# okieraised/rs-face-detection-tflite

Measured on AMD Instinct MI355X. Metric: faces/sec at batch=256 (256x256 back-camera) per GPU, higher is better.
Workload: dtype f32

## Files before the change

rs-face-detection-tflite_amd/csrc/engine.cpp:

```cpp
#include "engine.hpp"
#include "launch.hpp"

#include <algorithm>
#include <cstdio>
#include <cstdlib>
#include <cstring>
#include <stdexcept>

namespace mi {

void hip_check(hipError_t e, const char* what) {
    if (e != hipSuccess) throw std::runtime_error(std::string(what) + ": " + hipGetErrorString(e));
}

namespace {
template <class T>
void upload(T*& dev, std::vector<T>& host, const char* what_alloc, const char* what_copy) {
    if (dev) hip_check(hipFree(dev), "hipFree");
    dev = nullptr;
    if (host.empty()) return;
    hip_check(hipMalloc(reinterpret_cast<void**>(&dev), host.size() * sizeof(T)), what_alloc);
    hip_check(hipMemcpy(dev, host.data(), host.size() * sizeof(T), hipMemcpyHostToDevice), what_copy);
    std::vector<T>().swap(host);
}
}

Model::Model(const uint8_t* bytes, size_t n, int device) : device_(device), blob_(bytes, bytes + n) {
    int count = 0;
    if (hipGetDeviceCount(&count) != hipSuccess || count <= 0)
        throw std::runtime_error("no HIP device visible: the MI355X kernels cannot run (no CPU fallback exists)");
    if (device < 0 || device >= count) throw std::runtime_error("device ordinal out of range");
    hip_check(hipSetDevice(device_), "hipSetDevice");
    hipDeviceProp_t prop;
    hip_check(hipGetDeviceProperties(&prop, device_), "hipGetDeviceProperties");
    if (std::string(prop.gcnArchName).rfind("gfx950", 0) != 0)
        throw std::runtime_error(std::string("kernels are built for gfx950 only; device is ") + prop.gcnArchName);
    hip_check(hipStreamCreateWithFlags(&stream_, hipStreamNonBlocking), "hipStreamCreate");
    rebuild();
}

Model::~Model() {
    hipSetDevice(device_);
    invalidate_graphs();
    if (d_weights_) hipFree(d_weights_);
    if (d_programs_) hipFree(d_programs_);
    if (d_tail_programs_) hipFree(d_tail_programs_);
    if (d_arena_) hipFree(d_arena_);
    if (d_small_) hipFree(d_small_);
    if (d_in_stage_) hipFree(d_in_stage_);
    free_bandnet();
    for (float* p : d_out_)
        if (p) hipFree(p);
    for (hipStream_t st : side_streams_) hipStreamDestroy(st);
    for (hipEvent_t ev : lane_events_) hipEventDestroy(ev);
    for (hipStream_t st : head_streams_) hipStreamDestroy(st);
    for (hipEvent_t ev : head_events_) if (ev) hipEventDestroy(ev);
    if (stream_) hipStreamDestroy(stream_);
}

void Model::invalidate_graphs() {
    if (!graphs_.empty()) (void)hipDeviceSynchronize();
    for (auto& kv : graphs_) hipGraphExecDestroy(kv.second);
    graphs_.clear();
}

struct Model::Option {
    enum { kReplan = 1,
           kFreeSmall = 2,
           kKeepGraphs = 4,
           kOneOf = 8,
           kKiB = 16 , kWriteOnly = 32, kReadOnly = 64,
           kBandGen = 128 };
    const char* key;
    int Model::*field;
    int lo, hi, flags;
};

const Model::Option* Model::find_option(const std::string& key) {
    using O = Option;
    constexpr int kMax = 0x7fffffff;
    static const Option table[] = {
        {"chunk", &Model::chunk_, 0, kMax, 0},
        {"graph", &Model::use_graph_, 0, 1, 0},
        {"fuse", &Model::fuse_level_, 0, 5, O::kReplan},
        {"res_budget", &Model::res_budget_, 16, 156, O::kReplan | O::kKiB},
        {"pipe", &Model::pipe_max_, 0, 4, O::kReplan},
        {"small_chain", &Model::small_chain_, 0, 64, O::kFreeSmall},
        {"pipe_rows", &Model::pipe_rows_, 1 << 1 | 1 << 2 | 1 << 4, 0, O::kOneOf},
        {"pipe_band", &Model::pipe_band_, 0, 4096, 0},
        {"strip", &Model::strip_, 0, 1, 0},
        {"stem_fuse", &Model::stem_fuse_, 0, 1, 0},
        {"stem_mfma", &Model::stem_mfma_, 0, 1, 0},
        {"pair_fuse", &Model::pair_fuse_, 0, 1, 0},
        {"mdb_band", &Model::mdb_band_, 0, 4096, 0},
        {"mchain", &Model::mchain_, 0, 1, 0},
        {"tail", &Model::tail_, 0, 1, O::kReplan},
        {"tail_pre", &Model::tail_pre_, 0, 2, 0},
        {"tail_g", &Model::tail_g_, 0, 64, 0},
        {"band", &Model::band_, 0, 2, O::kReplan},
        {"band_test_fail", &Model::band_test_fail_, 0, 1, O::kWriteOnly},
        {"band_test_absent", &Model::band_test_absent_, 0, 256, O::kWriteOnly},
        {"band_test_gen", nullptr, 0, kMax, O::kBandGen | O::kWriteOnly},
        {"band_wide", &Model::band_wide_ok_, 0, 1, O::kReplan},
        {"band_fork", &Model::band_fork_, 0, 1, O::kReplan},
        {"band_nw", &Model::band_nw_, 8, 256, O::kReplan},
        {"band_fail_streak", &Model::band_fail_streak_, 0, 0, O::kReadOnly},
        {"band_wraps", &Model::band_wraps_, 0, 0, O::kReadOnly},
        {"fork", &Model::fork_, 0, 1, 0},
        {"heads", &Model::head_streams_opt_, 1, kHeadStreams, O::kReplan},
        {"reuse", &Model::reuse_, 0, 1, O::kReplan},
        {"lanes", &Model::lanes_, 1, 4, 0},
        {"test_poison", &Model::test_poison_, 1 << 1 | 1 << 2, 0, O::kOneOf | O::kKeepGraphs},
    };
    for (const Option& o : table)
        if (key == o.key) return &o;
    return nullptr;
}

void Model::set_option(const std::string& key, int value) {
    const Option* o = find_option(key);
    if (!o || (o->flags & Option::kReadOnly)) throw std::runtime_error("unknown option '" + key + "'");
    int v = (o->lo == 0 && o->hi == 1) ? value != 0 : std::min(o->hi, std::max(o->lo, value));
    if (o->flags & Option::kOneOf) v = (value >= 0 && value < 31 && (o->lo >> value & 1)) ? value : 0;
    if (o->flags & Option::kKiB) v *= 1024;
    if (o->flags & Option::kBandGen) { band_gen_ = static_cast<unsigned>(v); band_gen_force_ = true; }
    else this->*o->field = v;
    if (o->flags & Option::kKeepGraphs) return;
    if (o->flags & Option::kReplan) dirty_ = true;
    if ((o->flags & Option::kFreeSmall) && d_small_) { hipFree(d_small_); d_small_ = nullptr; small_floats_ = 0; }
    invalidate_graphs();
    chunk_cap_ = 0;
}

int Model::get_option(const std::string& key) const {
    const Option* o = find_option(key);
    if (!o || (o->flags & Option::kWriteOnly)) throw std::runtime_error("unknown option '" + key + "'");
    const int v = this->*o->field;
    return (o->flags & Option::kKiB) ? v / 1024 : v;
}

void Model::rebuild() {
    if (d_small_) { hipFree(d_small_); d_small_ = nullptr; small_floats_ = 0; }
    hip_check(hipSetDevice(device_), "hipSetDevice");
    invalidate_graphs();
    plan_ = build_plan(parse_tflite(blob_.data(), blob_.size()), fuse_level_, pipe_max_, res_budget_, tail_ != 0);
    if (!reuse_) {
        long off = 0;
        for (size_t t = 0; t < plan_.graph.tensors.size(); t++)
            if (plan_.root_offset[t] >= 0) { plan_.root_offset[t] = off; off += plan_.root_elems[t]; }
        plan_.arena_floats_per_frame = off;
    }
    consts_ = pack_plan_consts(plan_);
    upload(d_weights_, consts_.blob, "hipMalloc weights", "upload weights");
    upload(d_tail_programs_, consts_.tail_progs, "hipMalloc programs", "upload programs");
    upload(d_programs_, consts_.progs, "hipMalloc programs", "upload programs");
    sched_ = schedule_side_streams(plan_, head_streams_opt_);
    build_bandnet();
    dirty_ = false;
    chunk_cap_ = 0;
}

void Model::free_bandnet() {
    if (d_band_prog_) hipFree(d_band_prog_);
    if (d_band_consts_) hipFree(d_band_consts_);
    if (d_band_ws_) hipFree(d_band_ws_);
    if (d_band_sync_) hipFree(d_band_sync_);
    if (h_band_fail_) hipHostFree(h_band_fail_);
    d_band_prog_ = nullptr; d_band_consts_ = nullptr; d_band_ws_ = nullptr; d_band_sync_ = nullptr; h_band_fail_ = nullptr; d_band_fail_ = nullptr;
    band_plan_ = BandPlan();
}

void Model::build_bandnet() {
    free_bandnet();
    if (!band_ || fuse_level_ < 2) return;
    BandOptions o;
    o.nw = band_nw_; o.wide = band_wide_ok_ != 0; o.fork = band_fork_ != 0; o.cu_count = device_cu_count();
// ... 97 lines not shown
        for (int c : {n.w, n.b, n.w2, n.b2, n.alpha}) weights += 4 * elems(c);
        double bytes = per_frame * batch + weights;
        const auto& si = g.tensors[n.in[0]].shape;
        const auto& so = g.tensors[n.out].shape;
        if (n.kind == Node::Conv) macs = elems(n.out) * n.KH * n.KW * si.back() * batch;
        if (n.kind == Node::Dw) macs = elems(n.out) * n.KH * n.KW * batch;
        if (n.kind == Node::Block) macs = elems(n.out) / so.back() * si.back() * ((n.w >= 0 ? 9 : 0) + so.back()) * batch;
        if (n.kind == Node::Resident) {
            for (int t : n.extra_out) bytes += 4 * elems(t) * batch;
            for (const Node& m : n.members) {
                const auto& mo = g.tensors[m.out].shape;
                const int Cm = g.tensors[m.in[0]].shape[3];
                if (m.kind == Node::Conv) macs += elems(m.out) * m.KH * m.KW * Cm * batch;
                else macs += static_cast<double>(mo[1]) * mo[2] * Cm * ((m.w >= 0 ? 9 : 0) + mo[3]) * batch;
                for (int c : {m.w, m.b, m.w2, m.b2, m.alpha}) bytes += 4 * elems(c);
            }
        }
        if (n.kind == Node::Chain) {
            for (int t : n.extra_out) bytes += 4 * elems(t) * batch;
            for (const Node& m : n.members) {
                const auto& mo = g.tensors[m.out].shape;
                macs += static_cast<double>(mo[1]) * mo[2] * g.tensors[m.in[0]].shape[3] * (9 + mo[3]) * batch;
            }
            for (const Node& m : n.members)
                for (int c : {m.w, m.b, m.w2, m.b2, m.alpha}) bytes += 4 * elems(c);
            for (const Node& m : n.head_nodes) {
                macs += elems(m.out) * g.tensors[m.in[0]].shape[3] * batch;
                for (int c : {m.w, m.b, m.w2, m.b2}) bytes += 4 * elems(c);
            }
        }
        st.bytes += bytes;
        st.macs += macs;
        auto dims = [](const std::vector<int>& sh) {
            std::string d;
            for (size_t q = 1; q < sh.size(); q++) d += (q > 1 ? "x" : "") + std::to_string(sh[q]);
            return d;
        };
        if (static_cast<int>(i) == first.launches[k].node) st.detail = dims(si) + "->";
        st.detail = st.detail.substr(0, st.detail.find("->") + 2) + dims(so);
    }
    return stats;
}

LaunchCtx Model::launch_ctx(const float* in, int chunk_start, int frames) const {
    LaunchCtx c;
    c.weights = d_weights_;
    c.arena = d_arena_ + static_cast<size_t>(plan_.arena_floats_per_frame) * chunk_cap_ * arena_lane_;
    c.in = in; c.out = d_out_.data();
    c.small = d_small_; c.small_floats = small_floats_;
    c.progs = d_programs_; c.tail_progs = d_tail_programs_;
    c.band_prog = d_band_prog_; c.band_consts = d_band_consts_; c.band_ws = d_band_ws_; c.band_sync = d_band_sync_; c.band_fail = d_band_fail_;
    c.chunk_cap = chunk_cap_; c.chunk_start = chunk_start; c.F = frames;
    c.u8_frames = u8_.frames; c.u8_lut = u8_.lut; c.u8_frame_bytes = u8_.frame_bytes; c.u8_row_bytes = u8_.row_bytes;
    c.strip = strip_; c.pair_fuse = pair_fuse_; c.stem_fuse = stem_fuse_; c.stem_mfma = stem_mfma_; c.mchain = mchain_;
    c.small_chain = small_chain_; c.lanes = lanes_;
    c.pipe_rows = pipe_rows_; c.pipe_band = pipe_band_; c.mdb_band = mdb_band_; c.tail_pre = tail_pre_; c.tail_g = tail_g_;
    c.fork = fork_ && lanes_ == 1;
    c.cu_count = device_cu_count();
    c.band = band_use_ && chunk_start == 0;
    c.band_test_absent = band_test_absent_;
    return c;
}

namespace {
int issue(const Launch& l, hipStream_t s) {
    auto many = [&](int (*f)(const BlockArgs*, int, void*)) { return f(l.blocks.data(), static_cast<int>(l.blocks.size()), s); };
    switch (l.to) {
        case Launcher::Conv: return launch_conv(std::get<ConvArgs>(l.args), s);
        case Launcher::HeadGemm: return launch_head_gemm(std::get<HeadGemmArgs>(l.args), s);
        case Launcher::Dw: return launch_dw(std::get<DwArgs>(l.args), s);
        case Launcher::Xc: return launch_xc(std::get<XcArgs>(l.args), s);
        case Launcher::Mdblock: return launch_mdblock(std::get<DblockArgs>(l.args), s);
        case Launcher::Dblock: return launch_dblock(std::get<DblockArgs>(l.args), s);
        case Launcher::Mbneck: return launch_mbneck(std::get<BneckArgs>(l.args), s);
        case Launcher::Bneck: return launch_bneck(std::get<BneckArgs>(l.args), s);
        case Launcher::Tail: return launch_tail(std::get<TailLaunch>(l.args), s);
        case Launcher::Resident: return launch_resident(std::get<ResLaunch>(l.args), s);
        case Launcher::Chain: return launch_chain(std::get<ChainArgs>(l.args), s);
        case Launcher::StripPipe: return many(launch_strip_pipe);
        case Launcher::MstripChain: return many(launch_mstrip_chain);
        case Launcher::SmallChain: {
            int rc = 0;
            for (size_t k = 0; k < l.blocks.size() && rc == 0; k++) rc = l.blocks[k].sh == 1 ? launch_strip(l.blocks[k], s) : launch_block(l.blocks[k], s);
            return rc;
        }
        case Launcher::Ms2: return launch_ms2(std::get<BlockArgs>(l.args), s);
        case Launcher::Mwalk: return launch_mwalk(std::get<BlockArgs>(l.args), s);
        case Launcher::Strip: return launch_strip(std::get<BlockArgs>(l.args), s);
        case Launcher::Mstrip: return launch_mstrip(std::get<BlockArgs>(l.args), s);
        case Launcher::Block: return launch_block(std::get<BlockArgs>(l.args), s);
        case Launcher::Add: return launch_add(std::get<EltArgs>(l.args), s);
        case Launcher::Act: return launch_act(std::get<EltArgs>(l.args), s);
        case Launcher::Maxpool: return launch_maxpool(std::get<EltArgs>(l.args), s);
        case Launcher::Padc: return launch_padc(std::get<EltArgs>(l.args), s);
        case Launcher::Resize2x: return launch_resize2x(std::get<EltArgs>(l.args), s);
        case Launcher::DepthToSpace: return launch_depth_to_space(std::get<EltArgs>(l.args), s);
        case Launcher::Bandnet: return launch_bandnet(std::get<BandLaunch>(l.args), s);
    }
    return 0;
}
}

void Model::enqueue_chunk(const float* in, int chunk_start, int F, hipStream_t trunk, std::vector<hipEvent_t>* marks, Lowered* keep) {
    LaunchCtx ctx = launch_ctx(in, chunk_start, F);
    if (marks) ctx.fork = false;
    Lowered low = lower_chunk(plan_, consts_, band_plan_, sched_, ctx, keep != nullptr);
    auto mark = [&] {
// ... 254 lines not shown
```

rs-face-detection-tflite_amd/csrc/engine.hpp:

```cpp
#pragma once

#include <hip/hip_runtime.h>

#include <map>
#include <memory>
#include <string>
#include <vector>

#include "bandplan.hpp"
#include "consts.hpp"
#include "launches.hpp"
#include "plan.hpp"

namespace mi {

void hip_check(hipError_t e, const char* what);

class Model {
   public:
    Model(const uint8_t* bytes, size_t n, int device);
    ~Model();
    Model(const Model&) = delete;
    Model& operator=(const Model&) = delete;

    int device() const { return device_; }
    const Graph& graph() const { return plan_.graph; }
    const Plan& plan() const { return plan_; }
    std::vector<int> input_dims() const { return plan_.graph.tensors[plan_.graph.inputs[0]].shape; }
    int num_outputs() const { return static_cast<int>(plan_.graph.outputs.size()); }
    const std::vector<int>& output_dims(int i) const { return plan_.graph.tensors[plan_.graph.outputs.at(i)].shape; }
    size_t output_elems(int i) const { return plan_.graph.tensors[plan_.graph.outputs.at(i)].elems(); }
    size_t input_elems() const { return plan_.graph.tensors[plan_.graph.inputs[0]].elems(); }

    void run_device(const float* in, int batch, hipStream_t stream, bool one_shot = false);
    bool band_failed();
    int get_option(const std::string& key) const;
    int band_workgroups(int batch);
    void run(const float* in, int batch, float* const* outs, int mem, hipStream_t stream);
    float* output_device(int i) const { return d_out_.at(i); }
    hipStream_t stream() const { return stream_; }
    bool takes_u8_input();
    void run_device_u8(const uint8_t* frames, long frame_bytes, int row_bytes, const float* lut, int batch, hipStream_t stream);

    struct LaunchStat {
        std::string kernel, detail;
        double ms = 0, bytes = 0, macs = 0;
    };
    std::vector<LaunchStat> profile(const float* in, int batch, int reps, hipStream_t stream);
    void set_option(const std::string& key, int value);
    size_t debug_tensor(int tensor, int frame, float* dst, size_t cap);
    std::string describe() const { return plan_.describe(); }

   private:
    void rebuild();
    struct Option;
    static const Option* find_option(const std::string& key);
    void build_bandnet();
    void free_bandnet();
    bool band_usable(int batch) const;
    void band_before_launch(hipStream_t s);
    void poison_scratch(hipStream_t s);
    void ensure_capacity(int batch);
    LaunchCtx launch_ctx(const float* in, int chunk_start, int frames) const;
    void enqueue_chunk(const float* in, int chunk_start, int frames, hipStream_t s, std::vector<hipEvent_t>* marks = nullptr, Lowered* keep = nullptr);
    void enqueue_all(const float* in, int batch, hipStream_t s);
    void invalidate_graphs();

    int device_ = 0;
    std::vector<uint8_t> blob_;
    Plan plan_;
    int fuse_level_ = 5, pipe_max_ = 4, tail_ = 1, reuse_ = 1;
    int res_budget_ = 156 * 1024;
    int chunk_ = 0, lanes_ = 1, use_graph_ = 1;
    int fork_ = 1, head_streams_opt_ = 1;
    int strip_ = 1, stem_fuse_ = 1, stem_mfma_ = 1, pair_fuse_ = 1, mchain_ = 1;
    int pipe_rows_ = 0, pipe_band_ = 0, mdb_band_ = 0;
    int tail_pre_ = 0, tail_g_ = 0;
    int arena_lane_ = 0;
    std::vector<hipStream_t> side_streams_;
    std::vector<hipEvent_t> lane_events_;
    SideSchedule sched_;
    std::vector<hipStream_t> head_streams_;
    std::vector<hipEvent_t> head_events_;
    bool dirty_ = true;

    float* d_weights_ = nullptr;
    PlanConsts consts_;
    int profile_inner_ = 1;

    ResStage* d_programs_ = nullptr;
    TailStage* d_tail_programs_ = nullptr;
    float* d_arena_ = nullptr;
    size_t arena_floats_ = 0;
    int chunk_cap_ = 0;
    int batch_cap_ = 0;
    std::vector<float*> d_out_;
    float* d_in_stage_ = nullptr;
    size_t in_stage_floats_ = 0;
    int last_chunk_frames_ = 0;

    int band_ = 1;
    int band_nw_ = 128;
    BandPlan band_plan_;
    bool band_use_ = false;
    bool band_ran_ = false;
    int band_test_fail_ = 0;
    int band_test_absent_ = 0;
    int test_poison_ = 0;
    int band_fail_streak_ = 0;
    bool band_disabled_ = false;
    unsigned band_gen_ = 0;
    bool band_gen_force_ = false;
    int band_wraps_ = 0;
    size_t band_ws_bytes_ = 0;
    int band_fork_ = 1, band_wide_ok_ = 1;
    BandPacked* d_band_prog_ = nullptr;
    float* d_band_consts_ = nullptr;
    float* d_band_ws_ = nullptr;
    unsigned* d_band_sync_ = nullptr;
    int* h_band_fail_ = nullptr;
    int* d_band_fail_ = nullptr;

    hipStream_t stream_ = nullptr;
    int small_chain_ = 16;
    float* d_small_ = nullptr;
    size_t small_floats_ = 0;
    struct GraphKey {
        const void* in;
// ... 24 lines not shown
```

rs-face-detection-tflite_amd/csrc/kernels.hip:

```cpp
#include <hip/hip_runtime.h>

#include <cstdint>
#include <cstdlib>
#include <algorithm>
#include <type_traits>
#include <utility>

#include "kernels.hpp"
#include "launch.hpp"
#include "roi_dev.hpp"

namespace mi {

__device__ __forceinline__ float apply_act(float v, int act, const float* __restrict__ alpha, int c) {
    switch (act) {
        case ACT_RELU: return v > 0.f ? v : 0.f;
        case ACT_RELU6: return v < 0.f ? 0.f : (v > 6.f ? 6.f : v);
        case ACT_PRELU: return v >= 0.f ? v : alpha[c] * v;
        default: return v;
    }
}

__device__ __forceinline__ float load_res(const Epilogue& ep, int b, int oy, int ox, int Wo, int c) {
    if (ep.res_mode == RES_NONE || c >= ep.res_C) return 0.f;
// ... 190 lines not shown
#pragma unroll
    for (int p = 0; p < PP; p++) {
        __syncthreads();
        if (relu) {
#pragma unroll
            for (int o = 0; o < CO; o += 4) {
                const v2f r0 = __builtin_elementwise_max(acc2[p][o >> 1] + v2f{bias[o], bias[o + 1]}, v2f{0.f, 0.f});
                const v2f r1 = __builtin_elementwise_max(acc2[p][(o >> 1) + 1] + v2f{bias[o + 2], bias[o + 3]}, v2f{0.f, 0.f});
                *reinterpret_cast<float4*>(otile + tid * OS + o) = make_float4(r0.x, r0.y, r1.x, r1.y);
            }
        } else {
#pragma unroll
            for (int o = 0; o < CO; o += 4) {
                float r[4];
#pragma unroll
                for (int e = 0; e < 4; e++) {
                    const float acc = (e & 1) ? acc2[p][(o + e) >> 1].y : acc2[p][(o + e) >> 1].x;
                    const float v = acc + bias[o + e];
                    const float sl = prelu ? al[o + e] : base_slope;
                    r[e] = fminf(fmaxf(v, 0.f) + sl * fminf(v, 0.f), hi);
                }
                *reinterpret_cast<float4*>(otile + tid * OS + o) = make_float4(r[0], r[1], r[2], r[3]);
            }
        }
        __syncthreads();
        for (int i = tid; i < 8 * TW * C4; i += 256) {
            int px = i / C4, c4 = i - px * C4;
            int y = ty0 + 8 * p + px / TW, x = tx0 + (px & (TW - 1));
            if (y < a.Ho && x < a.Wo)
                *reinterpret_cast<float4*>(a.out + (long)b * a.out_fs + ((long)y * a.Wo + x) * CO_ALL + cs0 + 4 * c4) =
                    *reinterpret_cast<const float4*>(otile + px * OS + 4 * c4);
        }
    }
}

typedef float sv4f __attribute__((ext_vector_type(4)));
typedef unsigned su4 __attribute__((ext_vector_type(4)));
typedef unsigned su3 __attribute__((ext_vector_type(3)));
__device__ __forceinline__ sv4f stem_mfma4(float a, float b, sv4f c, int blk) {
    switch (blk) {
#define MI_SM4(N) case N: return __builtin_amdgcn_mfma_f32_4x4x1f32(a, b, c, 4, N, 0);
        MI_SM4(0) MI_SM4(1) MI_SM4(2) MI_SM4(3) MI_SM4(4) MI_SM4(5) MI_SM4(6) MI_SM4(7) MI_SM4(8) MI_SM4(9) MI_SM4(10) MI_SM4(11) MI_SM4(12) MI_SM4(13) MI_SM4(14)
#undef MI_SM4
        default: return __builtin_amdgcn_mfma_f32_4x4x1f32(a, b, c, 4, 15, 0);
    }
}

template <int N, class F, int... KS>
__device__ __forceinline__ void dfor_tiles_impl(F&& f, std::integer_sequence<int, KS...>) { (f(std::integral_constant<int, KS>{}), ...); }
template <int N, class F>
__device__ __forceinline__ void dfor_tiles(F&& f) { dfor_tiles_impl<N>(f, std::make_integer_sequence<int, N>{}); }

template <bool RELU>
__global__ __launch_bounds__(256) void stem_mfma_kernel(ConvArgs a, int tiles, int tpr) {
    constexpr int KW3 = 15, NK = 75, CQ = 6, NA = (NK * CQ + 15) / 16;
    const int lane = threadIdx.x & 63;
    const int G = (int)gridDim.x, wg = (G & 7) ? (int)blockIdx.x : (int)(blockIdx.x & 7) * (G >> 3) + (int)(blockIdx.x >> 3);
    const int wv = __builtin_amdgcn_readfirstlane(wg * 4 + (int)(threadIdx.x >> 6)), nwv = G * 4;
    float wa[NA];
#pragma unroll
    for (int r = 0; r < NA; r++) {
        const int n = 16 * r + (lane >> 2), k = n / CQ, t = n - CQ * k;
        wa[r] = n < NK * CQ ? a.w[k * 24 + 4 * t + (lane & 3)] : 0.f;
    }
    const float hi = a.ep.act == ACT_RELU6 ? 6.f : INFINITY, base_slope = a.ep.act == ACT_NONE ? 1.f : 0.f;
    const bool prelu = a.ep.act == ACT_PRELU;
    float bs[24], sl[RELU ? 1 : 24];
    {
        const float* __restrict__ bias = a.ep.bias;
        const float* __restrict__ al = prelu ? a.ep.alpha : a.ep.bias;
#pragma unroll
        for (int i = 0; i < 24; i++) bs[i] = bias[i];
        if constexpr (!RELU) {
#pragma unroll
            for (int i = 0; i < 24; i++) sl[i] = prelu ? al[i] : base_slope;
        }
    }
    const int rowb = a.W * 12;
    __shared__ __attribute__((aligned(16))) float otile[4 * 64 * 24];
    struct Tile { int b, y, half, px, lane_off; bool left, right; };
    auto setup = [&](int t) {
        Tile c;
        c.b = t / (a.Ho * tpr);
        const int rem = t - c.b * (a.Ho * tpr);
        c.y = rem / tpr; c.half = rem - c.y * tpr;
        c.px = 64 * c.half + lane;
        c.left = c.px == 0; c.right = c.px == a.Wo - 1;
        c.lane_off = (2 * c.px - 1 + (c.left ? 1 : 0) - (c.right ? 2 : 0)) * 12;
        return c;
    };
    auto load_row = [&](const Tile& c, int ky, float (&x)[KW3]) {
        const __amdgpu_buffer_rsrc_t rs = __builtin_amdgcn_make_buffer_rsrc(const_cast<float*>(a.in + (long)c.b * a.in_fs), 0, a.H * rowb, 0x00020000);
        const int vo = (2 * c.y - 1 + ky) * rowb + c.lane_off;
        const su4 q0 = __builtin_amdgcn_raw_buffer_load_b128(rs, vo, 0, 0), q1 = __builtin_amdgcn_raw_buffer_load_b128(rs, vo + 16, 0, 0),
                  q2 = __builtin_amdgcn_raw_buffer_load_b128(rs, vo + 32, 0, 0);
        const su3 q3 = __builtin_amdgcn_raw_buffer_load_b96(rs, vo + 48, 0, 0);
        x[0] = __uint_as_float(q0.x); x[1] = __uint_as_float(q0.y); x[2] = __uint_as_float(q0.z); x[3] = __uint_as_float(q0.w);
        x[4] = __uint_as_float(q1.x); x[5] = __uint_as_float(q1.y); x[6] = __uint_as_float(q1.z); x[7] = __uint_as_float(q1.w);
        x[8] = __uint_as_float(q2.x); x[9] = __uint_as_float(q2.y); x[10] = __uint_as_float(q2.z); x[11] = __uint_as_float(q2.w);
        x[12] = __uint_as_float(q3.x); x[13] = __uint_as_float(q3.y); x[14] = __uint_as_float(q3.z);
    };
    constexpr int NB = 2;
    float xb[NB][KW3];
    auto tile = [&](auto pc, const Tile& c, const Tile& nx) {
        constexpr int P = decltype(pc)::value;
        sv4f D[CQ];
#pragma unroll
        for (int q = 0; q < CQ; q++) D[q] = sv4f{0.f, 0.f, 0.f, 0.f};
#pragma unroll
        for (int ky = 0; ky < 5; ky++) {
            if (ky + NB - 1 < 5) load_row(c, ky + NB - 1, xb[(ky + NB - 1 + P) % NB]);
            else load_row(nx, ky + NB - 1 - 5, xb[(ky + NB - 1 + P) % NB]);
            float (&x)[KW3] = xb[(ky + P) % NB];
            if (c.half == 0) {
#pragma unroll
                for (int e = KW3 - 1; e >= 0; e--) x[e] = c.left ? (e >= 3 ? x[e - 3] : 0.f) : x[e];
            }
            if (c.half == tpr - 1) {
#pragma unroll
                for (int e = 0; e < KW3; e++) x[e] = c.right ? (e < 9 ? x[e + 6] : 0.f) : x[e];
            }
#pragma unroll
            for (int e = 0; e < KW3; e++)
#pragma unroll
                for (int q = 0; q < CQ; q++) {
                    const int n = (ky * KW3 + e) * CQ + q;
                    D[q] = stem_mfma4(wa[n >> 4], x[e], D[q], n & 15);
                }
        }
        float* ot = otile + (threadIdx.x >> 6) * (64 * 24);
#pragma unroll
        for (int q = 0; q < CQ; q++) {
            float r[4] = {D[q].x, D[q].y, D[q].z, D[q].w};
#pragma unroll
            for (int i = 0; i < 4; i++) {
                const float v = r[i] + bs[4 * q + i];
                if constexpr (RELU) r[i] = fmaxf(v, 0.f);
                else r[i] = fminf(fmaxf(v, 0.f) + sl[4 * q + i] * fminf(v, 0.f), hi);
            }
            *reinterpret_cast<float4*>(ot + lane * 24 + 4 * q) = make_float4(r[0], r[1], r[2], r[3]);
        }
        __builtin_amdgcn_wave_barrier();
        float* op = a.out + (long)c.b * a.out_fs + ((long)c.y * a.Wo + 64 * c.half) * 24;
#pragma unroll
        for (int q = 0; q < CQ; q++)
            *reinterpret_cast<float4*>(op + (q * 64 + lane) * 4) = *reinterpret_cast<const float4*>(ot + (q * 64 + lane) * 4);
        __builtin_amdgcn_wave_barrier();
    };
    if (wv >= tiles) return;
    Tile tl[2];
    tl[0] = setup(wv);
#pragma unroll
    for (int r = 0; r < NB - 1; r++) load_row(tl[0], r, xb[r]);
    for (int t = wv;;) {
        bool done = false;
        dfor_tiles<NB>([&](auto kc) {
            constexpr int k = decltype(kc)::value;
            if (done) return;
            const int tn = t + nwv;
            tl[(k + 1) & 1] = setup(min(tn, tiles - 1));
            tile(std::integral_constant<int, (5 * k) % NB>{}, tl[k & 1], tl[(k + 1) & 1]);
            if (tn >= tiles) done = true;
            t = tn;
        });
        if (done) break;
        if constexpr (NB & 1) { const Tile sw = tl[0]; tl[0] = tl[1]; tl[1] = sw; }
    }
}

static bool stem_mfma_applicable(const ConvArgs& a) {
    static const bool off = getenv("MI_NO_STEM_MFMA") != nullptr;
    if (off || a.no_mfma || a.in_u8 || a.KH != 5 || a.KW != 5 || a.C != 3 || a.Co != 24 || a.Cop != 24 || a.sh != 2 || a.sw != 2 || a.pt != 1 || a.pl != 1) return false;
    if (a.W != 2 * a.Wo || a.H != 2 * a.Ho || a.Wo % 64 || a.W < 8 || !a.ep.bias || a.ep.res_mode != RES_NONE) return false;
    if ((reinterpret_cast<uintptr_t>(a.in) & 15) || (a.in_fs & 3) || (reinterpret_cast<uintptr_t>(a.out) & 15) || (a.out_fs & 3)) return false;
    if ((long)a.H * a.W * 12 > 0x7fffffffL) return false;
    return (long)a.B * a.Ho * (a.Wo / 64) >= 64;
}

static int launch_stem_mfma(const ConvArgs& a, hipStream_t s) {
    const int tpr = a.Wo / 64, tiles = a.B * a.Ho * tpr;
    const int per_cu = 4;
    unsigned grid = (unsigned)std::min<long>((tiles + 3) / 4, (long)per_cu * device_cu_count());
    if (grid >= 64) grid &= ~7u;
    if (a.ep.act == ACT_RELU) return (int)launch_kernel(stem_mfma_kernel<true>, dim3(grid), dim3(256), 0, s, a, tiles, tpr);
    return (int)launch_kernel(stem_mfma_kernel<false>, dim3(grid), dim3(256), 0, s, a, tiles, tpr);
}

template <int K, int CO>
static int launch_stem(const ConvArgs& a, hipStream_t s) {
    constexpr int TH = 16;
    unsigned tiles = (unsigned)(((a.Wo + 31) / 32) * ((a.Ho + TH - 1) / TH));
    if (a.in_u8) return (int)launch_kernel(stem_conv_kernel<K, CO, true>, dim3(tiles * (unsigned)a.B), dim3(256), 0, s, a);
    constexpr int CS = CO == 64 ? 4 : CO / 8;
    const unsigned tiles1 = (unsigned)(((a.Wo + 31) / 32) * ((a.Ho + 7) / 8));
    if (tiles1 * (unsigned)a.B * CS <= 256u) return (int)launch_kernel(stem_conv_kernel<K, CO, false, CS, 1>, dim3(tiles1 * (unsigned)a.B * CS), dim3(256), 0, s, a);
    if (tiles * (unsigned)a.B * CS <= 256u) return (int)launch_kernel(stem_conv_kernel<K, CO, false, CS>, dim3(tiles * (unsigned)a.B * CS), dim3(256), 0, s, a);
    return (int)launch_kernel(stem_conv_kernel<K, CO, false>, dim3(tiles * (unsigned)a.B), dim3(256), 0, s, a);
}

static bool stem_applicable(const ConvArgs& a) {
    if (a.C != 3 || a.sh != 2 || a.sw != 2 || a.KH != a.KW || !a.ep.bias || a.ep.res_mode != RES_NONE) return false;
    if ((reinterpret_cast<uintptr_t>(a.out) & 15) || (a.out_fs & 3)) return false;
    return (a.KH == 5 && a.Co == 24) || (a.KH == 3 && (a.Co == 16 || a.Co == 32 || a.Co == 64));
}

static bool pw_few_applicable(const ConvArgs& a) {
    return a.KH == 1 && a.KW == 1 && a.sh == 1 && a.sw == 1 && a.Cop == 4 && a.C % 4 == 0 && a.H == a.Ho && a.W == a.Wo && (a.in_fs & 3) == 0 &&
           (reinterpret_cast<uintptr_t>(a.in) & 15) == 0 && (reinterpret_cast<uintptr_t>(a.w) & 15) == 0;
}
bool conv_takes_u8(const ConvArgs& a) { return stem_applicable(a); }
const char* conv_kernel_label(const ConvArgs& a) { return stem_applicable(a) ? (stem_mfma_applicable(a) ? "stem_mfma_kernel" : "stem_conv_kernel") : (pw_few_applicable(a) ? "pw_few_kernel" : "conv_generic_kernel"); }

int launch_conv(const ConvArgs& a, void* stream) {
    if (stem_applicable(a)) {
        hipStream_t st = (hipStream_t)stream;
        if (stem_mfma_applicable(a)) return launch_stem_mfma(a, st);
        if (a.KH == 5) return launch_stem<5, 24>(a, st);
        if (a.Co == 16) return launch_stem<3, 16>(a, st);
        if (a.Co == 32) return launch_stem<3, 32>(a, st);
        return launch_stem<3, 64>(a, st);
    }
    long total = (long)a.B * a.Ho * a.Wo * (a.Cop >> 2);
    if (total <= 0) return 0;
    unsigned blocks = (unsigned)((total + 255) / 256);
    if (pw_few_applicable(a)) return (int)launch_kernel(pw_few_kernel, dim3(blocks), dim3(256), 0, (hipStream_t)stream, a);
    return (int)launch_kernel(conv_generic_kernel, dim3(blocks), dim3(256), 0, (hipStream_t)stream, a);
}

template <int V>
__global__ __launch_bounds__(256) void dw_kernel(DwArgs a) {
    const int G = a.C / V;
    long idx = (long)blockIdx.x * blockDim.x + threadIdx.x;
    long total = (long)a.B * a.Ho * a.Wo * G;
    if (idx >= total) return;
    int g = (int)(idx % G);
    long p = idx / G;
    int ox = (int)(p % a.Wo);
    long q = p / a.Wo;
// ... 470 lines not shown
```

rs-face-detection-tflite_amd/csrc/kernels.hpp:

```cpp
#pragma once

#include <cstddef>
#include <cstdint>

namespace mi {

enum ActKind : int { ACT_NONE = 0, ACT_RELU = 1, ACT_RELU6 = 2, ACT_PRELU = 3 };
enum ResMode : int { RES_NONE = 0, RES_DIRECT = 1, RES_MAXPOOL = 2, RES_UP2X = 3 };

struct Epilogue {
    const float* bias = nullptr;
    const float* alpha = nullptr;
    const float* res = nullptr;
    long res_fs = 0;
    int res_mode = RES_NONE;
    int res_C = 0;
    int res_W = 0, res_H = 0;
    int act = ACT_NONE;
    int res_after = 0;
};

struct ConvArgs {
    const float* in = nullptr;
    const uint8_t* in_u8 = nullptr;
    const float* u8_lut = nullptr;
    long u8_frame_bytes = 0;
    int u8_row_bytes = 0;
    const float* w = nullptr;
    float* out = nullptr;
    long in_fs = 0, out_fs = 0;
    int B = 0, H = 0, W = 0, C = 0, Ho = 0, Wo = 0, Co = 0, Cop = 0;
    int KH = 1, KW = 1, sh = 1, sw = 1, pt = 0, pl = 0;
    Epilogue ep;
    int no_mfma = 0;
};

struct HeadGemmArgs {
    const float* in = nullptr;
    const float* w = nullptr;
    const float* bias = nullptr;
    const float* alpha = nullptr;
    float* out = nullptr;
    long in_fs = 0, out_fs = 0;
    int B = 0, K = 0, N = 0;
    int act = ACT_NONE;
};

struct DwArgs {
    const float* in = nullptr;
    const float* w = nullptr;
    float* out = nullptr;
    long in_fs = 0, out_fs = 0;
    int B = 0, H = 0, W = 0, C = 0, Ho = 0, Wo = 0;
    int KH = 3, KW = 3, sh = 1, sw = 1, pt = 0, pl = 0;
    Epilogue ep;
};

struct BlockArgs {
    const float* in = nullptr;
    const float* w_dw = nullptr;
    const float* b_dw = nullptr;
    const float* w_pw = nullptr;
    const float* w_strip = nullptr;
    const float* w_mwalk = nullptr;
    float* out = nullptr;
    long in_fs = 0, out_fs = 0;
    int B = 0, H = 0, W = 0, C = 0, Ho = 0, Wo = 0, Co = 0;
    int sh = 1, sw = 1, pt = 0, pl = 0;
    int has_dw = 1;
    int pipe_rows = 0;
    int pipe_band = 0;
    Epilogue ep;
};

constexpr int kMaxChain = 8;
struct ChainBlock {
    const float* w_dw = nullptr;
    const float* b_dw = nullptr;
    const float* w_pw = nullptr;
    const float* bias = nullptr;
    const float* alpha = nullptr;
    int act = ACT_NONE;
    int has_res = 0;
};
struct ChainEdge {
    int on = 0;
    ChainBlock blk;
// ... 376 lines not shown
```

rs-face-detection-tflite_amd/csrc/launches.cpp:

```cpp
#include "launches.hpp"

#include <algorithm>
#include <cmath>
#include <cstdio>
#include <cstdlib>
#include <stdexcept>

namespace mi {

namespace {
void same_pad(int in, int k, int stride, int out, int* before) { *before = std::max(0, (out - 1) * stride + k - in) / 2; }
bool is_view(const Node& n) { return n.kind == Node::Reshape || n.kind == Node::Concat; }
int dim(const std::vector<int>& v, size_t d) { return d < v.size() ? v[d] : 1; }
float clamp_of(int act) { return act == ACT_RELU6 ? 6.f : INFINITY; }
}

bool band_cut(const BandPlan& bp, size_t i) { return static_cast<int>(i) >= bp.first && !bp.node_runs[i]; }

int band_run_launches(const Plan& plan, const BandPlan& bp) {
    int launches = 1;
    for (size_t i = 0; i < plan.nodes.size(); i++)
        if (!is_view(plan.nodes[i]) && !band_cut(bp, i)) launches++;
    return launches;
}
// ... 249 lines not shown
                } else if (n.kind == Node::Pad) {
                    const auto& pv = g.tensors[n.pads].i32;
                    if (pv[0] != 0 || pv[1] != 0) throw std::runtime_error("PAD on the batch axis unsupported");
                    a.p0 = pv[2]; a.p1 = pv[4]; a.p2 = pv[6];
                    set(l, Launcher::Padc, a, lab("pad_kernel"));
                } else if (n.kind == Node::Resize) {
                    a.p0 = n.half_pixel; a.p1 = n.align_corners;
                    set(l, Launcher::Resize2x, a, lab("resize_kernel"));
                } else if (n.kind == Node::DepthToSpace) {
                    a.p0 = n.block_size;
                    set(l, Launcher::DepthToSpace, a, lab("d2s_kernel"));
                } else {
                    throw std::runtime_error("internal: unhandled node kind");
                }
                return 1;
            }
        }
    }

    size_t conv(size_t i, Launch& l, const Epilogue& ep, const float* ip, long in_fs, float* op, long out_fs) const {
        const Node& n = plan.nodes[i];
        const auto& si = shape(n.in[0]);
        const auto& so = shape(n.out);
        if (n.gemm_head) {
            HeadGemmArgs h;
            h.in = ip; h.out = op; h.in_fs = in_fs; h.out_fs = out_fs;
            h.w = c.weights + pc.node_w[i];
            h.bias = ep.bias; h.alpha = ep.alpha; h.act = ep.act;
            h.B = c.F; h.K = si[1] * si[2] * si[3]; h.N = so[3];
            set(l, Launcher::HeadGemm, h, lab(c.F <= 4 ? "head_dot_kernel" : "head_gemm_kernel"));
            return 1;
        }
        if (c.strip && c.stem_fuse && pc.node_stem[i] >= 0 && !c.u8_frames) {
            const size_t j = i + 1;
            if (pc.node_chain_pair[j] >= 0 && !sched.event_after[i] && sched.slot[j] < 0) {
                const Node& ch = plan.nodes[j];
                DblockArgs d = dblock_args(nullptr, 0, n.out, ch.out, ch.members[0], ch.members[1], pc.node_chain_pair[j], true);
                d.stem_in = ip; d.stem_in_fs = in_fs; d.stem_consts = c.weights + pc.node_stem[i];
                d.stem_hi = clamp_of(n.act);
                if (mdblock_kernel_supports(d)) {
                    set(l, Launcher::Mdblock, d, lab("mdblock_kernel<stem+pair>"));
                    return 2;
                }
            }
        }
        ConvArgs a;
        a.in = ip; a.out = op; a.in_fs = in_fs; a.out_fs = out_fs;
        a.w = c.weights + pc.node_w[i];
        a.B = c.F; a.H = si[1]; a.W = si[2]; a.C = si[3]; a.Ho = so[1]; a.Wo = so[2]; a.Co = so[3]; a.Cop = (a.Co + 3) & ~3;
        a.KH = n.KH; a.KW = n.KW; a.sh = n.sh; a.sw = n.sw;
        if (n.padding == Padding::Same) { same_pad(a.H, a.KH, a.sh, a.Ho, &a.pt); same_pad(a.W, a.KW, a.sw, a.Wo, &a.pl); }
        if (n.ept >= 0) { a.pt = n.ept; a.pl = n.epl; }
        a.ep = ep;
        a.no_mfma = c.stem_mfma ? 0 : 1;
        if (c.u8_frames && plan.storage[n.in[0]].root == plan.storage[g.inputs[0]].root) {
            if (!conv_takes_u8(a)) throw std::runtime_error("plan: this graph's first convolution has no u8 input form");
            a.in_u8 = c.u8_frames + static_cast<long>(c.chunk_start) * c.u8_frame_bytes;
            a.u8_lut = c.u8_lut; a.u8_frame_bytes = c.u8_frame_bytes; a.u8_row_bytes = c.u8_row_bytes;
        }
        set(l, Launcher::Conv, a, want_labels ? conv_kernel_label(a) : nullptr);
        return 1;
    }

    void resident(size_t i, Launch& l, const float* ip, long in_fs, float* op, long out_fs) const {
        const Node& n = plan.nodes[i];
        const auto& si = shape(n.in[0]);
        if (n.xc) {
            XcArgs a;
            a.in = ip; a.in_fs = in_fs; a.out = op; a.out_fs = out_fs;
            a.B = c.F; a.H = si[1]; a.W = si[2]; a.nstages = static_cast<int>(n.members.size());
            for (size_t k = 0; k < n.members.size(); k++) {
                const Node& m = n.members[k];
                const MemberOff& mo = pc.chain_off[i][k];
                XcStage& st = a.st[k];
                st.cblob = c.weights + mo.cblob;
                st.has_dw = m.w >= 0;
                st.w_pw = c.weights + mo.w2;
                st.C = shape(m.in[0])[3]; st.Co = shape(m.out)[3]; st.act = m.act;
                st.skip = m.res < 0 ? 0 : (m.res == m.in[0] ? 1 : (k >= 2 && m.res == n.members[k - 2].out ? 3 : 2));
                if (st.skip == 2) {
                    st.res = tensor_ptr(m.res, &st.res_fs);
                    st.res_C = shape(m.res)[3]; st.res_W = shape(m.res)[2];
                }
            }
            return set(l, Launcher::Xc, a, lab("xc_kernel"));
        }
        if (n.dblock) {
            DblockArgs a = dblock_args(ip, in_fs, n.in[0], n.out, n.members[0], n.members[1], pc.chain_off[i][1].mconsts, false);
            a.w1 = c.weights + pc.chain_off[i][0].w2;
            a.w2 = c.weights + pc.chain_off[i][1].w2;
            a.consts = c.weights + pc.chain_off[i][0].cblob;
            if (c.strip && mdblock_kernel_supports(a)) return set(l, Launcher::Mdblock, a, lab("mdblock_kernel"));
            return set(l, Launcher::Dblock, a, lab("dblock_kernel"));
        }
        if (n.bneck) {
            BneckArgs a;
            a.in = ip; a.in_fs = in_fs; a.out = op; a.out_fs = out_fs;
            a.B = c.F; a.H = si[1]; a.W = si[2]; a.C = si[3]; a.Cm = shape(n.members[0].out)[3];
            a.nblocks = static_cast<int>(n.members.size() / 2);
            a.bands = n.res_bands;
            for (int k = 0; k < a.nblocks; k++) {
                const size_t ka = static_cast<size_t>(2 * k), kb = ka + 1;
                const MemberOff &ma = pc.chain_off[i][ka], &mb = pc.chain_off[i][kb];
                a.blocks[k].w1 = c.weights + ma.w2;
                a.blocks[k].w2 = c.weights + mb.w2;
                a.blocks[k].consts = c.weights + ma.cblob;
                a.blocks[k].hi1 = clamp_of(n.members[ka].act);
// ... 248 lines not shown
```

rs-face-detection-tflite_amd/csrc/launches.hpp:

```cpp
#pragma once

#include <string>
#include <variant>
#include <vector>

#include "bandplan.hpp"
#include "consts.hpp"
#include "kernels.hpp"
#include "plan.hpp"

namespace mi {

constexpr int kHeadStreams = 4;

struct SideSchedule {
    std::vector<int> slot, wait;
    std::vector<char> event_after;
};
SideSchedule schedule_side_streams(const Plan& plan, int head_streams);

struct LaunchCtx {
    const float* weights = nullptr;
    float* arena = nullptr;
    const float* in = nullptr;
    float* const* out = nullptr;
    float* small = nullptr;
    size_t small_floats = 0;
    const ResStage* progs = nullptr;
    const TailStage* tail_progs = nullptr;
    const BandPacked* band_prog = nullptr;
    const float* band_consts = nullptr;
    float* band_ws = nullptr;
    unsigned* band_sync = nullptr;
    int* band_fail = nullptr;
    int chunk_cap = 0, chunk_start = 0, F = 0;
    const uint8_t* u8_frames = nullptr;
    const float* u8_lut = nullptr;
    long u8_frame_bytes = 0;
    int u8_row_bytes = 0;
    int strip = 1, pair_fuse = 1, stem_fuse = 1, stem_mfma = 1, mchain = 1, small_chain = 16, lanes = 1;
    int pipe_rows = 0, pipe_band = 0, mdb_band = 0, tail_pre = 0, tail_g = 0;
    bool fork = true;
    int cu_count = 256;
    bool band = false;
    int band_test_absent = 0;
};

enum class Launcher {
    Conv, HeadGemm, Dw, Xc, Mdblock, Dblock, Mbneck, Bneck, Tail, Resident, Chain, StripPipe, SmallChain, Ms2, Mwalk, MstripChain, Strip, Mstrip, Block,
    Add, Act, Maxpool, Padc, Resize2x, DepthToSpace, Bandnet
};

struct Launch {
    Launcher to = Launcher::Conv;
    std::variant<ConvArgs, HeadGemmArgs, DwArgs, XcArgs, DblockArgs, BneckArgs, TailLaunch, ResLaunch, ChainArgs, BlockArgs, EltArgs, BandLaunch> args;
    std::vector<BlockArgs> blocks;
    int node = -1, last = -1;
    int slot = -1;
    int wait = -1;
    bool record = false;
    std::string label;
};

struct Lowered {
    std::vector<Launch> launches;
    std::vector<int> launch_of_node;
};
Lowered lower_chunk(const Plan& plan, const PlanConsts& consts, const BandPlan& band_plan, const SideSchedule& sched, const LaunchCtx& ctx, bool want_labels);

float* tensor_ptr_mut(const Plan& plan, const LaunchCtx& ctx, int t, long* frame_stride);

bool band_cut(const BandPlan& band_plan, size_t i);
int band_run_launches(const Plan& plan, const BandPlan& band_plan);

bool takes_u8_input(const Plan& plan, const PlanConsts& consts);

}
```

Before: 212,300.

## Add row-run stem MFMA kernel reusing input rows across outputs

Adds a stem convolution kernel in which each wave walks a run of R consecutive output rows. It keeps a rotating five-row register buffer, so each output row needs only two new input rows instead of five. R is picked automatically from tile count and CU count, or set through a new stem_run option. The previous per-tile kernel stays selectable via stem_mfma=2. Per-wave serial work grows and the grid shrinks, which may reduce latency hiding.

```diff
diff --git a/rs-face-detection-tflite_amd/csrc/engine.cpp b/rs-face-detection-tflite_amd/csrc/engine.cpp
--- a/rs-face-detection-tflite_amd/csrc/engine.cpp
+++ b/rs-face-detection-tflite_amd/csrc/engine.cpp
@@ -70,7 +70,8 @@
            kKeepGraphs = 4,
            kOneOf = 8,
            kKiB = 16 , kWriteOnly = 32, kReadOnly = 64,
-           kBandGen = 128 };
+           kBandGen = 128,
+           kForms = 256 };
     const char* key;
     int Model::*field;
     int lo, hi, flags;
@@ -90,7 +91,8 @@
         {"pipe_band", &Model::pipe_band_, 0, 4096, 0},
         {"strip", &Model::strip_, 0, 1, 0},
         {"stem_fuse", &Model::stem_fuse_, 0, 1, 0},
-        {"stem_mfma", &Model::stem_mfma_, 0, 1, 0},
+        {"stem_mfma", &Model::stem_mfma_, 0, 2, O::kForms},
+        {"stem_run", &Model::stem_run_, 0, 32, 0},
         {"pair_fuse", &Model::pair_fuse_, 0, 1, 0},
         {"mdb_band", &Model::mdb_band_, 0, 4096, 0},
         {"mchain", &Model::mchain_, 0, 1, 0},
@@ -122,6 +124,7 @@
     if (!o || (o->flags & Option::kReadOnly)) throw std::runtime_error("unknown option '" + key + "'");
     int v = (o->lo == 0 && o->hi == 1) ? value != 0 : std::min(o->hi, std::max(o->lo, value));
     if (o->flags & Option::kOneOf) v = (value >= 0 && value < 31 && (o->lo >> value & 1)) ? value : 0;
+    if (o->flags & Option::kForms) v = (value >= o->lo && value <= o->hi) ? value : 1;
     if (o->flags & Option::kKiB) v *= 1024;
     if (o->flags & Option::kBandGen) { band_gen_ = static_cast<unsigned>(v); band_gen_force_ = true; }
     else this->*o->field = v;
@@ -325,7 +328,7 @@
     c.band_prog = d_band_prog_; c.band_consts = d_band_consts_; c.band_ws = d_band_ws_; c.band_sync = d_band_sync_; c.band_fail = d_band_fail_;
     c.chunk_cap = chunk_cap_; c.chunk_start = chunk_start; c.F = frames;
     c.u8_frames = u8_.frames; c.u8_lut = u8_.lut; c.u8_frame_bytes = u8_.frame_bytes; c.u8_row_bytes = u8_.row_bytes;
-    c.strip = strip_; c.pair_fuse = pair_fuse_; c.stem_fuse = stem_fuse_; c.stem_mfma = stem_mfma_; c.mchain = mchain_;
+    c.strip = strip_; c.pair_fuse = pair_fuse_; c.stem_fuse = stem_fuse_; c.stem_mfma = stem_mfma_; c.stem_run = stem_run_; c.mchain = mchain_;
     c.small_chain = small_chain_; c.lanes = lanes_;
     c.pipe_rows = pipe_rows_; c.pipe_band = pipe_band_; c.mdb_band = mdb_band_; c.tail_pre = tail_pre_; c.tail_g = tail_g_;
     c.fork = fork_ && lanes_ == 1;
diff --git a/rs-face-detection-tflite_amd/csrc/engine.hpp b/rs-face-detection-tflite_amd/csrc/engine.hpp
--- a/rs-face-detection-tflite_amd/csrc/engine.hpp
+++ b/rs-face-detection-tflite_amd/csrc/engine.hpp
@@ -73,7 +73,7 @@
     int res_budget_ = 156 * 1024;
     int chunk_ = 0, lanes_ = 1, use_graph_ = 1;
     int fork_ = 1, head_streams_opt_ = 1;
-    int strip_ = 1, stem_fuse_ = 1, stem_mfma_ = 1, pair_fuse_ = 1, mchain_ = 1;
+    int strip_ = 1, stem_fuse_ = 1, stem_mfma_ = 1, stem_run_ = 0, pair_fuse_ = 1, mchain_ = 1;
     int pipe_rows_ = 0, pipe_band_ = 0, mdb_band_ = 0;
     int tail_pre_ = 0, tail_g_ = 0;
     int arena_lane_ = 0;
diff --git a/rs-face-detection-tflite_amd/csrc/kernels.hip b/rs-face-detection-tflite_amd/csrc/kernels.hip
--- a/rs-face-detection-tflite_amd/csrc/kernels.hip
+++ b/rs-face-detection-tflite_amd/csrc/kernels.hip
@@ -266,7 +266,7 @@
 __device__ __forceinline__ void dfor_tiles(F&& f) { dfor_tiles_impl<N>(f, std::make_integer_sequence<int, N>{}); }
 
 template <bool RELU>
-__global__ __launch_bounds__(256) void stem_mfma_kernel(ConvArgs a, int tiles, int tpr) {
+__global__ __launch_bounds__(256) void stem_mfma_rowwise_kernel(ConvArgs a, int tiles, int tpr) {
     constexpr int KW3 = 15, NK = 75, CQ = 6, NA = (NK * CQ + 15) / 16;
     const int lane = threadIdx.x & 63;
     const int G = (int)gridDim.x, wg = (G & 7) ? (int)blockIdx.x : (int)(blockIdx.x & 7) * (G >> 3) + (int)(blockIdx.x >> 3);
@@ -306,6 +306,11 @@
     auto load_row = [&](const Tile& c, int ky, float (&x)[KW3]) {
         const __amdgpu_buffer_rsrc_t rs = __builtin_amdgcn_make_buffer_rsrc(const_cast<float*>(a.in + (long)c.b * a.in_fs), 0, a.H * rowb, 0x00020000);
         const int vo = (2 * c.y - 1 + ky) * rowb + c.lane_off;
+#ifdef MI_ABL_STEM_NOLOAD
+#pragma unroll
+        for (int e = 0; e < KW3; e++) x[e] = wa[e + (vo & 1)];
+        return;
+#endif
         const su4 q0 = __builtin_amdgcn_raw_buffer_load_b128(rs, vo, 0, 0), q1 = __builtin_amdgcn_raw_buffer_load_b128(rs, vo + 16, 0, 0),
                   q2 = __builtin_amdgcn_raw_buffer_load_b128(rs, vo + 32, 0, 0);
         const su3 q3 = __builtin_amdgcn_raw_buffer_load_b96(rs, vo + 48, 0, 0);
@@ -334,6 +339,10 @@
 #pragma unroll
                 for (int e = 0; e < KW3; e++) x[e] = c.right ? (e < 9 ? x[e + 6] : 0.f) : x[e];
             }
+#ifdef MI_ABL_STEM_NOMFMA
+#pragma unroll
+            for (int e = 0; e < KW3; e++) D[e % CQ].x += x[e];
+#else
 #pragma unroll
             for (int e = 0; e < KW3; e++)
 #pragma unroll
@@ -341,6 +350,7 @@
                     const int n = (ky * KW3 + e) * CQ + q;
                     D[q] = stem_mfma4(wa[n >> 4], x[e], D[q], n & 15);
                 }
+#endif
         }
         float* ot = otile + (threadIdx.x >> 6) * (64 * 24);
 #pragma unroll
@@ -356,6 +366,9 @@
         }
         __builtin_amdgcn_wave_barrier();
         float* op = a.out + (long)c.b * a.out_fs + ((long)c.y * a.Wo + 64 * c.half) * 24;
+#ifdef MI_ABL_STEM_NOSTORE
+        if (a.B >= 0) return;
+#endif
 #pragma unroll
         for (int q = 0; q < CQ; q++)
             *reinterpret_cast<float4*>(op + (q * 64 + lane) * 4) = *reinterpret_cast<const float4*>(ot + (q * 64 + lane) * 4);
@@ -382,9 +395,115 @@
     }
 }
 
+template <bool RELU>
+__global__ __launch_bounds__(256) void stem_mfma_kernel(ConvArgs a, int runs, int R) {
+    constexpr int KW3 = 15, NK = 75, CQ = 6, NA = (NK * CQ + 15) / 16, NR = 5;
+    const int lane = threadIdx.x & 63;
+    const int G = (int)gridDim.x, wg = (G & 7) ? (int)blockIdx.x : (int)(blockIdx.x & 7) * (G >> 3) + (int)(blockIdx.x >> 3);
+    const int wv = __builtin_amdgcn_readfirstlane(wg * 4 + (int)(threadIdx.x >> 6)), nwv = G * 4;
+    if (wv >= runs) return;
+    float wa[NA];
+#pragma unroll
+    for (int r = 0; r < NA; r++) {
+        const int n = 16 * r + (lane >> 2), k = n / CQ, t = n - CQ * k;
+        wa[r] = n < NK * CQ ? a.w[k * 24 + 4 * t + (lane & 3)] : 0.f;
+    }
+    const float hi = a.ep.act == ACT_RELU6 ? 6.f : INFINITY, base_slope = a.ep.act == ACT_NONE ? 1.f : 0.f;
+    const bool prelu = a.ep.act == ACT_PRELU;
+    float bs[24], sl[RELU ? 1 : 24];
+    {
+        const float* __restrict__ bias = a.ep.bias;
+        const float* __restrict__ al = prelu ? a.ep.alpha : a.ep.bias;
+#pragma unroll
+        for (int i = 0; i < 24; i++) bs[i] = bias[i];
+        if constexpr (!RELU) {
+#pragma unroll
+            for (int i = 0; i < 24; i++) sl[i] = prelu ? al[i] : base_slope;
+        }
+    }
+    const int rowb = a.W * 12, tpr = a.Wo >> 6, rpf = ((a.Ho + R - 1) / R) * tpr;
+    __shared__ __attribute__((aligned(16))) float otile[4 * 64 * 24];
+    float* const ot = otile + (threadIdx.x >> 6) * (64 * 24);
+    float xb[NR][KW3];
+    for (int run = wv; run < runs; run += nwv) {
+        const int b = run / rpf, rem = run - b * rpf, half = rem % tpr, y0 = (rem / tpr) * R, yend = min(y0 + R, a.Ho);
+        const int px = 64 * half + lane;
+        const bool left = px == 0, right = px == a.Wo - 1, has_left = half == 0, has_right = half == tpr - 1;
+        const int lane_off = (2 * px - 1 + (left ? 1 : 0) - (right ? 2 : 0)) * 12;
+        const __amdgpu_buffer_rsrc_t rs = __builtin_amdgcn_make_buffer_rsrc(const_cast<float*>(a.in + (long)b * a.in_fs), 0, a.H * rowb, 0x00020000);
+        auto load_row = [&](int row, float (&x)[KW3]) {
+            const int vo = (int)((unsigned)row * (unsigned)rowb + (unsigned)lane_off);
+            const su4 q0 = __builtin_amdgcn_raw_buffer_load_b128(rs, vo, 0, 0), q1 = __builtin_amdgcn_raw_buffer_load_b128(rs, vo + 16, 0, 0),
+                      q2 = __builtin_amdgcn_raw_buffer_load_b128(rs, vo + 32, 0, 0);
+            const su3 q3 = __builtin_amdgcn_raw_buffer_load_b96(rs, vo + 48, 0, 0);
+            x[0] = __uint_as_float(q0.x); x[1] = __uint_as_float(q0.y); x[2] = __uint_as_float(q0.z); x[3] = __uint_as_float(q0.w);
+            x[4] = __uint_as_float(q1.x); x[5] = __uint_as_float(q1.y); x[6] = __uint_as_float(q1.z); x[7] = __uint_as_float(q1.w);
+            x[8] = __uint_as_float(q2.x); x[9] = __uint_as_float(q2.y); x[10] = __uint_as_float(q2.z); x[11] = __uint_as_float(q2.w);
+            x[12] = __uint_as_float(q3.x); x[13] = __uint_as_float(q3.y); x[14] = __uint_as_float(q3.z);
+        };
+        auto fix_edges = [&](float (&x)[KW3]) {
+            if (has_left) {
+#pragma unroll
+                for (int e = KW3 - 1; e >= 0; e--) x[e] = left ? (e >= 3 ? x[e - 3] : 0.f) : x[e];
+            }
+            if (has_right) {
+#pragma unroll
+                for (int e = 0; e < KW3; e++) x[e] = right ? (e < 9 ? x[e + 6] : 0.f) : x[e];
+            }
+        };
+#pragma unroll
+        for (int ky = 0; ky < NR; ky++) load_row(2 * y0 - 1 + ky, xb[ky]);
+#pragma unroll
+        for (int ky = 0; ky < 3; ky++) fix_edges(xb[ky]);
+        float* op = a.out + (long)b * a.out_fs + ((long)y0 * a.Wo + 64 * half) * 24;
+        for (int y = y0;;) {
+            bool done = false;
+            dfor_tiles<NR>([&](auto sc) {
+                constexpr int S = decltype(sc)::value;
+                if (done) return;
+                sv4f D[CQ];
+#pragma unroll
+                for (int q = 0; q < CQ; q++) D[q] = sv4f{0.f, 0.f, 0.f, 0.f};
+#pragma unroll
+                for (int ky = 0; ky < NR; ky++) {
+                    float (&x)[KW3] = xb[(ky + 2 * S) % NR];
+                    if (ky >= 3) fix_edges(x);
+#pragma unroll
+                    for (int e = 0; e < KW3; e++)
+#pragma unroll
+                        for (int q = 0; q < CQ; q++) {
+                            const int n = (ky * KW3 + e) * CQ + q;
+                            D[q] = stem_mfma4(wa[n >> 4], x[e], D[q], n & 15);
+                        }
+                    if (ky < 2) load_row(2 * y + 4 + ky, x);
+                }
+#pragma unroll
+                for (int q = 0; q < CQ; q++) {
+                    float r[4] = {D[q].x, D[q].y, D[q].z, D[q].w};
+#pragma unroll
+                    for (int i = 0; i < 4; i++) {
+                        const float v = r[i] + bs[4 * q + i];
+                        if constexpr (RELU) r[i] = fmaxf(v, 0.f);
+                        else r[i] = fminf(fmaxf(v, 0.f) + sl[4 * q + i] * fminf(v, 0.f), hi);
+                    }
+                    *reinterpret_cast<float4*>(ot + lane * 24 + 4 * q) = make_float4(r[0], r[1], r[2], r[3]);
+                }
+                __builtin_amdgcn_wave_barrier();
+#pragma unroll
+                for (int q = 0; q < CQ; q++)
+                    *reinterpret_cast<float4*>(op + (q * 64 + lane) * 4) = *reinterpret_cast<const float4*>(ot + (q * 64 + lane) * 4);
+                __builtin_amdgcn_wave_barrier();
+                op += a.Wo * 24;
+                if (++y >= yend) done = true;
+            });
+            if (done) break;
+        }
+    }
+}
+
 static bool stem_mfma_applicable(const ConvArgs& a) {
     static const bool off = getenv("MI_NO_STEM_MFMA") != nullptr;
-    if (off || a.no_mfma || a.in_u8 || a.KH != 5 || a.KW != 5 || a.C != 3 || a.Co != 24 || a.Cop != 24 || a.sh != 2 || a.sw != 2 || a.pt != 1 || a.pl != 1) return false;
+    if (off || a.no_mfma == 1 || a.in_u8 || a.KH != 5 || a.KW != 5 || a.C != 3 || a.Co != 24 || a.Cop != 24 || a.sh != 2 || a.sw != 2 || a.pt != 1 || a.pl != 1) return false;
     if (a.W != 2 * a.Wo || a.H != 2 * a.Ho || a.Wo % 64 || a.W < 8 || !a.ep.bias || a.ep.res_mode != RES_NONE) return false;
     if ((reinterpret_cast<uintptr_t>(a.in) & 15) || (a.in_fs & 3) || (reinterpret_cast<uintptr_t>(a.out) & 15) || (a.out_fs & 3)) return false;
     if ((long)a.H * a.W * 12 > 0x7fffffffL) return false;
@@ -393,11 +512,23 @@
 
 static int launch_stem_mfma(const ConvArgs& a, hipStream_t s) {
     const int tpr = a.Wo / 64, tiles = a.B * a.Ho * tpr;
+    const int run_cu = 2;
+    int R = a.stem_run;
+    if (R <= 0 && a.no_mfma == 0)
+        for (R = 1; R < 32 && (long)tiles >= 2L * R * 4 * run_cu * device_cu_count(); R *= 2) {}
+    if (a.no_mfma == 0 && (R >= 2 || a.stem_run > 0)) {
+        R = std::min(R, a.Ho);
+        const int runs = a.B * ((a.Ho + R - 1) / R) * tpr;
+        unsigned grid = (unsigned)std::min<long>((runs + 3) / 4, (long)run_cu * device_cu_count());
+        if (grid >= 64) grid &= ~7u;
+        if (a.ep.act == ACT_RELU) return (int)launch_kernel(stem_mfma_kernel<true>, dim3(grid), dim3(256), 0, s, a, runs, R);
+        return (int)launch_kernel(stem_mfma_kernel<false>, dim3(grid), dim3(256), 0, s, a, runs, R);
+    }
     const int per_cu = 4;
     unsigned grid = (unsigned)std::min<long>((tiles + 3) / 4, (long)per_cu * device_cu_count());
     if (grid >= 64) grid &= ~7u;
-    if (a.ep.act == ACT_RELU) return (int)launch_kernel(stem_mfma_kernel<true>, dim3(grid), dim3(256), 0, s, a, tiles, tpr);
-    return (int)launch_kernel(stem_mfma_kernel<false>, dim3(grid), dim3(256), 0, s, a, tiles, tpr);
+    if (a.ep.act == ACT_RELU) return (int)launch_kernel(stem_mfma_rowwise_kernel<true>, dim3(grid), dim3(256), 0, s, a, tiles, tpr);
+    return (int)launch_kernel(stem_mfma_rowwise_kernel<false>, dim3(grid), dim3(256), 0, s, a, tiles, tpr);
 }
 
 template <int K, int CO>
diff --git a/rs-face-detection-tflite_amd/csrc/kernels.hpp b/rs-face-detection-tflite_amd/csrc/kernels.hpp
--- a/rs-face-detection-tflite_amd/csrc/kernels.hpp
+++ b/rs-face-detection-tflite_amd/csrc/kernels.hpp
@@ -33,6 +33,7 @@
     int KH = 1, KW = 1, sh = 1, sw = 1, pt = 0, pl = 0;
     Epilogue ep;
     int no_mfma = 0;
+    int stem_run = 0;
 };
 
 struct HeadGemmArgs {
diff --git a/rs-face-detection-tflite_amd/csrc/launches.cpp b/rs-face-detection-tflite_amd/csrc/launches.cpp
--- a/rs-face-detection-tflite_amd/csrc/launches.cpp
+++ b/rs-face-detection-tflite_amd/csrc/launches.cpp
@@ -325,7 +325,8 @@
         if (n.padding == Padding::Same) { same_pad(a.H, a.KH, a.sh, a.Ho, &a.pt); same_pad(a.W, a.KW, a.sw, a.Wo, &a.pl); }
         if (n.ept >= 0) { a.pt = n.ept; a.pl = n.epl; }
         a.ep = ep;
-        a.no_mfma = c.stem_mfma ? 0 : 1;
+        a.no_mfma = c.stem_mfma == 0 ? 1 : c.stem_mfma == 2 ? 2 : 0;
+        a.stem_run = c.stem_run;
         if (c.u8_frames && plan.storage[n.in[0]].root == plan.storage[g.inputs[0]].root) {
             if (!conv_takes_u8(a)) throw std::runtime_error("plan: this graph's first convolution has no u8 input form");
             a.in_u8 = c.u8_frames + static_cast<long>(c.chunk_start) * c.u8_frame_bytes;
diff --git a/rs-face-detection-tflite_amd/csrc/launches.hpp b/rs-face-detection-tflite_amd/csrc/launches.hpp
--- a/rs-face-detection-tflite_amd/csrc/launches.hpp
+++ b/rs-face-detection-tflite_amd/csrc/launches.hpp
@@ -38,7 +38,7 @@
     const float* u8_lut = nullptr;
     long u8_frame_bytes = 0;
     int u8_row_bytes = 0;
-    int strip = 1, pair_fuse = 1, stem_fuse = 1, stem_mfma = 1, mchain = 1, small_chain = 16, lanes = 1;
+    int strip = 1, pair_fuse = 1, stem_fuse = 1, stem_mfma = 1, stem_run = 0, mchain = 1, small_chain = 16, lanes = 1;
     int pipe_rows = 0, pipe_band = 0, mdb_band = 0, tail_pre = 0, tail_g = 0;
     bool fork = true;
     int cu_count = 256;
```

After: 214,600 (median of 6 runs). 1.01x the previous value.
